# Tcadart/pyLatticeDSO

Hardware: AMD Instinct MI355X
Metric: beams/s assembly+PCG-solve (higher is better)
Workload: dtype f64

## Files before the change

### pylatticedso_amd/csrc/pl_coarse.h

```cpp
#pragma once
#include <hip/hip_runtime.h>

#include <algorithm>
#include <cstdint>
#include <cstdlib>
#include <vector>

#include "pl_dense.h"
#include "pl_kernels.h"
#include "pl_nodeword.h"
#include "pl_tile.h"

namespace pl {

constexpr int kDclMax = 256;
constexpr int kDclSlots = 4096;
inline bool node_words_enabled() {
  const char *e = std::getenv("PL_NODE_WORDS");
  return !(e && e[0] == '0');
}

struct Coarse {
  bool enabled = false;
  bool ready = false;
// ... 1380 lines not shown
                                                                 const double *__restrict__ xyz,
                                                                 const int32_t *__restrict__ agg_of_tile,
                                                                 const double *__restrict__ cen,
                                                                 const double *__restrict__ yc,
                                                                 const double *__restrict__ yt ,
                                                                 const uint8_t *__restrict__ fixedbits,
                                                                 PT *__restrict__ p, RT *__restrict__ x,
                                                                 const double *__restrict__ scal,
                                                                 double *__restrict__ scal_next,
                                                                 double *__restrict__ hist, int k,
                                                                 double *__restrict__ rc, int ncp,
                                                                 const int32_t *__restrict__ aggL_of_tile ,
                                                                 const double *__restrict__ cenL,
                                                                 const double *__restrict__ ycL,
                                                                 const uint8_t *__restrict__ shared ,
                                                                 double *__restrict__ rcL, int ncpL,
                                                                 const uint8_t *__restrict__ zero_rows ,
                                                                 int cm = 6,
                                                                 const float *__restrict__ rel32 = nullptr ,
                                                                 const uint32_t *__restrict__ nword = nullptr,
                                                                 const uint32_t *__restrict__ dtab = nullptr,
                                                                 double rscale = 0.0 ) {
  if constexpr (!MULTI) shared = nullptr;
  if constexpr (!MULTI || !LOCAL) aggL_of_tile = nullptr;
  double old, rz_new, pap;
  scalar_read3(scal, S_RZ_OLD, S_RZ_NEW, S_PAP, old, rz_new, pap);
  const double beta = (old != 0.0) ? rz_new / old : 0.0;
  const double alpha = (pap != 0.0) ? old / pap : 0.0;
  if (blockIdx.x == 1 || gridDim.x == 1)
    for (int e = threadIdx.x; e < ncp; e += blockDim.x) rc[e] = 0.0;
  if (aggL_of_tile && (blockIdx.x == 2 || gridDim.x <= 2))
    for (int e = threadIdx.x; e < ncpL; e += blockDim.x) rcL[e] = 0.0;
  if (blockIdx.x == 0 && threadIdx.x < kWave) {
    const int s = threadIdx.x;
    double rr = 0.0;
    for (int q = s; q < kSlots; q += kWave) rr += rc[ncp + q];
    rr = wave_sum(rr);
    if (s == 0) hist[k] = rr;
    for (int q = s; q < kSlots; q += kWave) {
      rc[ncp + q] = 0.0;
      rc[ncp + kSlots + q] = 0.0;
      scal_next[S_RZ_OLD * kSlots + q] = scal[S_RZ_NEW * kSlots + q];
      scal_next[S_RZ_NEW * kSlots + q] = 0.0;
      scal_next[S_PAP * kSlots + q] = 0.0;
    }
  }
  const int t = blockIdx.x;
  const int n0 = tile_start[t], n1 = tile_start[t + 1];
  const int a = agg_of_tile[t];
  const double *y = yc + cm * a;
  double U0 = y[0], U1 = y[1], U2 = y[2], W0 = y[3], W1 = y[4], W2 = y[5];
  double T[TM];
#pragma unroll
  for (int k = 0; k < TM; ++k) T[k] = 0.0;
  if (yt) {
    const double *q = yt + TM * (size_t)t;
#pragma unroll
    for (int k = 0; k < TM; ++k) T[k] = q[k];
    if (!shared) {
      U0 += T[0]; U1 += T[1]; U2 += T[2]; W0 += T[3]; W1 += T[4]; W2 += T[5];
    }
  }
  double ED[6] = {0, 0, 0, 0, 0, 0};
  if constexpr (TM == 12) {
    if (cm == 12) {
#pragma unroll
      for (int k = 0; k < 6; ++k) ED[k] = y[6 + k];
      if (!shared) {
#pragma unroll
        for (int k = 0; k < 6; ++k) {
          T[6 + k] += ED[k];
          ED[k] = 0.0;
        }
      }
    }
  }
  const bool own_t = yt && shared;
  const double c0 = cen[3 * a], c1 = cen[3 * a + 1], c2 = cen[3 * a + 2];
  double L[6] = {0, 0, 0, 0, 0, 0}, l0 = 0.0, l1 = 0.0, l2 = 0.0;
  if (aggL_of_tile) {
    const int aL = aggL_of_tile[t];
#pragma unroll
    for (int q = 0; q < 6; ++q) L[q] = ycL[6 * aL + q];
    l0 = cenL[3 * aL];
    l1 = cenL[3 * aL + 1];
    l2 = cenL[3 * aL + 2];
  }
  for (int64_t i = n0 + threadIdx.x; i < n1; i += blockDim.x) {
    if (zero_rows && zero_rows[i]) continue;
    const uint32_t nw = nword ? nword[i] : 0u;
    double rx, ry, rz;
    if (rscale != 0.0) {
      nword_rel(nw, rscale, rx, ry, rz);
    } else if (rel32) {
      rx = (double)rel32[3 * i];
      ry = (double)rel32[3 * i + 1];
      rz = (double)rel32[3 * i + 2];
    } else {
      rx = xyz[3 * i] - c0;
      ry = xyz[3 * i + 1] - c1;
      rz = xyz[3 * i + 2] - c2;
    }
    double zc[6] = {U0 + (W1 * rz - W2 * ry), U1 + (W2 * rx - W0 * rz), U2 + (W0 * ry - W1 * rx), W0, W1, W2};
    if constexpr (TM == 12) {
     if (shared && cm == 12) {
      zc[0] += ED[0] * rx + 0.5 * (ED[3] * ry + ED[5] * rz);
      zc[1] += ED[1] * ry + 0.5 * (ED[3] * rx + ED[4] * rz);
      zc[2] += ED[2] * rz + 0.5 * (ED[4] * ry + ED[5] * rx);
     }
     if (!(shared && shared[i])) {
      zc[0] += T[6] * rx + 0.5 * (T[9] * ry + T[11] * rz);
      zc[1] += T[7] * ry + 0.5 * (T[9] * rx + T[10] * rz);
      zc[2] += T[8] * rz + 0.5 * (T[10] * ry + T[11] * rx);
     }
    }
    if (own_t && !shared[i]) {
      zc[0] += T[0] + (T[4] * rz - T[5] * ry);
      zc[1] += T[1] + (T[5] * rx - T[3] * rz);
      zc[2] += T[2] + (T[3] * ry - T[4] * rx);
      zc[3] += T[3];
      zc[4] += T[4];
      zc[5] += T[5];
    }
    if (aggL_of_tile && !(shared && shared[i])) {
      const double sx = xyz[3 * i] - l0, sy = xyz[3 * i + 1] - l1, sz = xyz[3 * i + 2] - l2;
      zc[0] += L[0] + (L[4] * sz - L[5] * sy);
      zc[1] += L[1] + (L[5] * sx - L[3] * sz);
      zc[2] += L[2] + (L[3] * sy - L[4] * sx);
      zc[3] += L[3];
      zc[4] += L[4];
      zc[5] += L[5];
    }
    const uint32_t *row = dtab ? dtab + 8 * (nw >> 24) : nullptr;
    const unsigned fb = dtab ? row[6] : (unsigned)fixedbits[i];
    const float2 *d2 = dtab ? reinterpret_cast<const float2 *>(row) : reinterpret_cast<const float2 *>(dinv32 + 6 * i);
#pragma unroll
    for (int q = 0; q < 3; ++q) {
      const double2 rr = load_pair(r, 3 * i + q);
      const float2 dd = d2[q];
      double2 pp = load_pair(p, 3 * i + q);
      double2 xx = load_pair(x, 3 * i + q);
      xx.x += alpha * pp.x;
      xx.y += alpha * pp.y;
      store_pair(x, 3 * i + q, xx);
      const double z0 = dd.x * rr.x + (((fb >> (2 * q)) & 1u) ? 0.0 : zc[2 * q]);
      const double z1 = dd.y * rr.y + (((fb >> (2 * q + 1)) & 1u) ? 0.0 : zc[2 * q + 1]);
      pp.x = z0 + beta * pp.x;
      pp.y = z1 + beta * pp.y;
      store_pair(p, 3 * i + q, pp);
    }
  }
}

template <typename PT, typename RT, int TM>
__global__ __launch_bounds__(kBlock) void k_pcg_direction_flat(int64_t N, const int32_t *__restrict__ tile_of_node,
                                                               const RT *__restrict__ r,
                                                               const float *__restrict__ dinv32,
                                                               const double *__restrict__ xyz,
                                                               const int32_t *__restrict__ agg_of_tile,
                                                               const double *__restrict__ cen,
                                                               const double *__restrict__ yc,
                                                               const double *__restrict__ yt ,
                                                               const uint8_t *__restrict__ fixedbits,
                                                               PT *__restrict__ p, RT *__restrict__ x,
                                                               const double *__restrict__ scal,
                                                               double *__restrict__ scal_next,
                                                               double *__restrict__ hist, int k,
                                                               double *__restrict__ rc, int ncp,
                                                               const int32_t *__restrict__ keep ,
                                                               int cm, const uint8_t *__restrict__ shared ,
                                                               const float *__restrict__ rel32 = nullptr ,
                                                               const uint32_t *__restrict__ nword = nullptr,
                                                               const uint32_t *__restrict__ dtab = nullptr,
                                                               double rscale = 0.0 ) {
  double old, rz_new, pap;
  scalar_read3(scal, S_RZ_OLD, S_RZ_NEW, S_PAP, old, rz_new, pap);
  const double beta = (old != 0.0) ? rz_new / old : 0.0;
  const double alpha = (pap != 0.0) ? old / pap : 0.0;
  if (blockIdx.x == 1 || gridDim.x == 1)
    for (int e = threadIdx.x; e < ncp; e += blockDim.x) rc[e] = 0.0;
  if (blockIdx.x == 0 && threadIdx.x < kWave) {
    const int s = threadIdx.x;
    double rr = 0.0;
    for (int q = s; q < kSlots; q += kWave) rr += rc[ncp + q];
    rr = wave_sum(rr);
    if (s == 0) hist[k] = rr;
    for (int q = s; q < kSlots; q += kWave) {
      rc[ncp + q] = 0.0;
      rc[ncp + kSlots + q] = 0.0;
      scal_next[S_RZ_OLD * kSlots + q] = scal[S_RZ_NEW * kSlots + q];
      scal_next[S_RZ_NEW * kSlots + q] = 0.0;
      scal_next[S_PAP * kSlots + q] = 0.0;
    }
  }
  const int64_t lane_pair = (int64_t)blockIdx.x * blockDim.x + threadIdx.x;
  if (lane_pair >= 3 * N) return;
  const int64_t slot = lane_pair / 3;
  const int q = (int)(lane_pair - 3 * slot);
  const int64_t i = keep ? (int64_t)keep[slot] : slot;
  const int64_t pair = 3 * i + q;
  const int t = tile_of_node[i];
  const int a = agg_of_tile[t];
  const double *y = yc + cm * a;
  double C[12];
#pragma unroll
  for (int m = 0; m < 6; ++m) C[m] = y[m];
#pragma unroll
  for (int m = 6; m < 12; ++m) C[m] = 0.0;
  if constexpr (TM == 12) {
    if (cm == 12) {
#pragma unroll
      for (int m = 6; m < 12; ++m) C[m] = y[m];
    }
  }
  if (yt && !(shared && shared[i])) {
    const double *w = yt + TM * (size_t)t;
#pragma unroll
    for (int m = 0; m < TM; ++m) C[m] += w[m];
  }
  const uint32_t nw = nword ? nword[i] : 0u;
  double rx, ry, rz;
  if (rscale != 0.0) {
    nword_rel(nw, rscale, rx, ry, rz);
  } else if (rel32) {
    rx = (double)rel32[3 * i];
    ry = (double)rel32[3 * i + 1];
    rz = (double)rel32[3 * i + 2];
  } else {
    rx = xyz[3 * i] - cen[3 * a];
    ry = xyz[3 * i + 1] - cen[3 * a + 1];
    rz = xyz[3 * i + 2] - cen[3 * a + 2];
  }
  double zc[6] = {C[0] + (C[4] * rz - C[5] * ry), C[1] + (C[5] * rx - C[3] * rz), C[2] + (C[3] * ry - C[4] * rx),
                  C[3], C[4], C[5]};
  if constexpr (TM == 12) {
    zc[0] += C[6] * rx + 0.5 * (C[9] * ry + C[11] * rz);
    zc[1] += C[7] * ry + 0.5 * (C[9] * rx + C[10] * rz);
    zc[2] += C[8] * rz + 0.5 * (C[10] * ry + C[11] * rx);
  }
  double z0 = q == 0 ? zc[0] : (q == 1 ? zc[2] : zc[4]);
  double z1 = q == 0 ? zc[1] : (q == 1 ? zc[3] : zc[5]);
  const uint32_t *row = dtab ? dtab + 8 * (nw >> 24) : nullptr;
  const unsigned fb = dtab ? row[6] : (unsigned)fixedbits[i];
  const float2 dd = dtab ? reinterpret_cast<const float2 *>(row)[q] : reinterpret_cast<const float2 *>(dinv32)[pair];
  const double2 rr = load_pair(r, pair);
  double2 pp = load_pair(p, pair);
  double2 xx = load_pair(x, pair);
  xx.x += alpha * pp.x;
  xx.y += alpha * pp.y;
  store_pair(x, pair, xx);
  z0 = dd.x * rr.x + (((fb >> (2 * q)) & 1u) ? 0.0 : z0);
  z1 = dd.y * rr.y + (((fb >> (2 * q + 1)) & 1u) ? 0.0 : z1);
  pp.x = z0 + beta * pp.x;
  pp.y = z1 + beta * pp.y;
  store_pair(p, pair, pp);
}

}
```

### pylatticedso_amd/csrc/pl_kernels.h

```cpp
#pragma once
#include "pl_device.h"

namespace pl {

constexpr int kBlock = 256;
constexpr int kWave = 64;
constexpr int kDefaultLPN = 4;
constexpr int kSlots = 64;

__device__ __forceinline__ unsigned xcd_block(unsigned b, unsigned nblk) {
  const unsigned xcd = b & 7u, q = nblk >> 3, r = nblk & 7u;
  const unsigned base = (xcd < r) ? xcd * (q + 1) : r * (q + 1) + (xcd - r) * q;
  return base + (b >> 3);
}

__device__ __forceinline__ double dpp_row_shr_add(double v, const int ctrl_tag) {
  int lo = __double2loint(v), hi = __double2hiint(v);
  switch (ctrl_tag) {
    case 1: lo = __builtin_amdgcn_update_dpp(0, lo, 0x111, 0xf, 0xf, true); hi = __builtin_amdgcn_update_dpp(0, hi, 0x111, 0xf, 0xf, true); break;
    case 2: lo = __builtin_amdgcn_update_dpp(0, lo, 0x112, 0xf, 0xf, true); hi = __builtin_amdgcn_update_dpp(0, hi, 0x112, 0xf, 0xf, true); break;
    case 4: lo = __builtin_amdgcn_update_dpp(0, lo, 0x114, 0xf, 0xf, true); hi = __builtin_amdgcn_update_dpp(0, hi, 0x114, 0xf, 0xf, true); break;
    default: lo = __builtin_amdgcn_update_dpp(0, lo, 0x118, 0xf, 0xf, true); hi = __builtin_amdgcn_update_dpp(0, hi, 0x118, 0xf, 0xf, true); break;
  }
  return v + __hiloint2double(hi, lo);
}
__device__ __forceinline__ double row_sums(double v) {
  v = dpp_row_shr_add(v, 1);
  v = dpp_row_shr_add(v, 2);
  v = dpp_row_shr_add(v, 4);
  return dpp_row_shr_add(v, 8);
}
__device__ __forceinline__ double lane_value(double v, int l) {
  return __hiloint2double(__builtin_amdgcn_readlane(__double2hiint(v), l), __builtin_amdgcn_readlane(__double2loint(v), l));
}
__device__ __forceinline__ double lane_value_dyn(double v, int l) {
  return __hiloint2double(__shfl(__double2hiint(v), l), __shfl(__double2loint(v), l));
}
__device__ __forceinline__ double wave_sum(double v) {
  v = dpp_row_shr_add(v, 1);
  v = dpp_row_shr_add(v, 2);
  v = dpp_row_shr_add(v, 4);
  v = dpp_row_shr_add(v, 8);
  const int lo = __double2loint(v), hi = __double2hiint(v);
  double t = __hiloint2double(__builtin_amdgcn_readlane(hi, 15), __builtin_amdgcn_readlane(lo, 15));
  t += __hiloint2double(__builtin_amdgcn_readlane(hi, 31), __builtin_amdgcn_readlane(lo, 31));
  t += __hiloint2double(__builtin_amdgcn_readlane(hi, 47), __builtin_amdgcn_readlane(lo, 47));
  t += __hiloint2double(__builtin_amdgcn_readlane(hi, 63), __builtin_amdgcn_readlane(lo, 63));
  return t;
}

__device__ __forceinline__ void scalar_add(double *scal, int which, double v) {
  unsafeAtomicAdd(scal + which * kSlots + (blockIdx.x & (kSlots - 1)), v);
}
__device__ __forceinline__ double scalar_read(const double *scal, int which) {
  const int lane = threadIdx.x & 63;
  double v = 0.0;
#pragma unroll
  for (int s = lane; s < kSlots; s += 64) v += scal[which * kSlots + s];
  return wave_sum(v);
}

__device__ __forceinline__ void scalar_read2(const double *scal, int a, int b, double &va, double &vb) {
  static_assert(kSlots == kWave, "one slot per lane");
  const int lane = threadIdx.x & 63;
  const double xa = scal[a * kSlots + lane], xb = scal[b * kSlots + lane];
  va = wave_sum(xa);
  vb = wave_sum(xb);
}
__device__ __forceinline__ void scalar_read3(const double *scal, int a, int b, int c, double &va, double &vb, double &vc) {
  static_assert(kSlots == kWave, "one slot per lane");
  const int lane = threadIdx.x & 63;
  const double xa = scal[a * kSlots + lane], xb = scal[b * kSlots + lane], xc = scal[c * kSlots + lane];
  va = wave_sum(xa);
  vb = wave_sum(xb);
  vc = wave_sum(xc);
}

__device__ __forceinline__ double block_sum(double v, double *smem ) {
  v = wave_sum(v);
  const int lane = threadIdx.x & 63, w = threadIdx.x >> 6;
  if (lane == 0) smem[w] = v;
  __syncthreads();
  double t = 0.0;
  if (threadIdx.x == 0) {
#pragma unroll
    for (int i = 0; i < kBlock / kWave; ++i) t += smem[i];
  }
  return t;
}

__device__ __forceinline__ void load6(const double *__restrict__ p, V3 &u, V3 &t) {
  const double2 *q = reinterpret_cast<const double2 *>(p);
  const double2 a = q[0], b = q[1], c = q[2];
  u = {a.x, a.y, b.x};
  t = {b.y, c.x, c.y};
}
__device__ __forceinline__ void store6(double *__restrict__ p, V3 u, V3 t) {
  double2 *q = reinterpret_cast<double2 *>(p);
  q[0] = {u.x, u.y};
  q[1] = {u.z, t.x};
  q[2] = {t.y, t.z};
}

__device__ __forceinline__ void load6(const float *__restrict__ p, V3 &u, V3 &t) {
  const float2 *q = reinterpret_cast<const float2 *>(p);
  const float2 a = q[0], b = q[1], c = q[2];
  u = {(double)a.x, (double)a.y, (double)b.x};
  t = {(double)b.y, (double)c.x, (double)c.y};
}
__device__ __forceinline__ double2 load_pair(const double *v, int64_t pair) {
  return reinterpret_cast<const double2 *>(v)[pair];
}
__device__ __forceinline__ double2 load_pair(const float *v, int64_t pair) {
  const float2 f = reinterpret_cast<const float2 *>(v)[pair];
  return {(double)f.x, (double)f.y};
}
__device__ __forceinline__ void store_pair(double *v, int64_t pair, double2 a) {
  reinterpret_cast<double2 *>(v)[pair] = a;
}
__device__ __forceinline__ void store_pair(float *v, int64_t pair, double2 a) {
  reinterpret_cast<float2 *>(v)[pair] = {(float)a.x, (float)a.y};
}

__device__ __forceinline__ Record load_record(const Record *__restrict__ rec, int64_t i) {
  const double2 *q = reinterpret_cast<const double2 *>(rec + i);
  const double2 a = q[0], b = q[1], c = q[2], d = q[3];
  Record r;
  r.a = a.x; r.c = a.y; r.e1 = b.x; r.e2 = b.y; r.e3 = c.x; r.dx = c.y; r.dy = d.x; r.dz = d.y;
  return r;
}

__global__ __launch_bounds__(kBlock) void k_build_records(int64_t B, const double *__restrict__ xyz,
                                                          const int32_t *__restrict__ conn,
                                                          const double *__restrict__ radius,
                                                          const double *__restrict__ seg_len,
                                                          const int32_t *__restrict__ seg_nsub,
                                                          const double *__restrict__ mult, Material m,
                                                          Record *__restrict__ rec, double *__restrict__ rec5) {
  const int64_t b = (int64_t)xcd_block(blockIdx.x, gridDim.x) * kBlock + threadIdx.x;
  if (b >= B) return;
  if (mult) m = scaled(m, mult[b]);
  const int ia = conn[2 * b], ib = conn[2 * b + 1];
  const V3 d = {xyz[3 * (int64_t)ib] - xyz[3 * (int64_t)ia], xyz[3 * (int64_t)ib + 1] - xyz[3 * (int64_t)ia + 1],
                xyz[3 * (int64_t)ib + 2] - xyz[3 * (int64_t)ia + 2]};
  const double len[3] = {seg_len[3 * b], seg_len[3 * b + 1], seg_len[3 * b + 2]};
  const int ns[3] = {seg_nsub[3 * b], seg_nsub[3 * b + 1], seg_nsub[3 * b + 2]};
  const Flex f = strut_flexibility(radius[b], len, ns, m);
  const Record r = make_record(scalars_from_flex(f), d);
  rec[b] = r;
  if (rec5) {
    double *q = rec5 + 5 * b;
    q[0] = r.a; q[1] = r.c; q[2] = r.e1; q[3] = r.e2; q[4] = r.e3;
  }
}

__global__ __launch_bounds__(kBlock) void k_spmv_atomic(int64_t B, const int32_t *__restrict__ conn,
                                                        const Record *__restrict__ rec, const double *__restrict__ x,
                                                        double *__restrict__ y) {
  const int64_t b = (int64_t)xcd_block(blockIdx.x, gridDim.x) * kBlock + threadIdx.x;
  if (b >= B) return;
  const int64_t ia = conn[2 * b], ib = conn[2 * b + 1];
  const Record r = load_record(rec, b);
  V3 uA, tA, uB, tB, F, M;
  load6(x + 6 * ia, uA, tA);
  load6(x + 6 * ib, uB, tB);
  tip_force(r, uA, tA, uB, tB, F, M);
  const V3 d = {r.dx, r.dy, r.dz};
  const V3 MA = (-1.0) * M - cross(d, F);
  double *ya = y + 6 * ia, *yb = y + 6 * ib;
  unsafeAtomicAdd(yb + 0, F.x); unsafeAtomicAdd(yb + 1, F.y); unsafeAtomicAdd(yb + 2, F.z);
  unsafeAtomicAdd(yb + 3, M.x); unsafeAtomicAdd(yb + 4, M.y); unsafeAtomicAdd(yb + 5, M.z);
  unsafeAtomicAdd(ya + 0, -F.x); unsafeAtomicAdd(ya + 1, -F.y); unsafeAtomicAdd(ya + 2, -F.z);
  unsafeAtomicAdd(ya + 3, MA.x); unsafeAtomicAdd(ya + 4, MA.y); unsafeAtomicAdd(ya + 5, MA.z);
}

__global__ __launch_bounds__(kBlock) void k_mask_dot(int64_t n6, const uint8_t *__restrict__ fixed,
                                                     const double *__restrict__ x, double *__restrict__ y,
                                                     double *__restrict__ dot_out) {
  __shared__ double red[kBlock / kWave];
  double acc = 0.0;
  for (int64_t i = (int64_t)blockIdx.x * kBlock + threadIdx.x; i < n6; i += (int64_t)gridDim.x * kBlock) {
    double v = y[i];
    if (fixed && fixed[i]) { v = 0.0; y[i] = 0.0; }
    acc += x[i] * v;
  }
  if (dot_out) {
    const double t = block_sum(acc, red);
    if (threadIdx.x == 0) unsafeAtomicAdd(dot_out + (blockIdx.x & (kSlots - 1)), t);
  }
}

template <int LPN>
__device__ __forceinline__ double lpn_sum(double v) {
#pragma unroll
  for (int o = kWave / LPN; o < kWave; o <<= 1) v += __shfl_xor(v, o, 64);
  return v;
}

template <int LPN, bool MASK, bool DOT>
__global__ __launch_bounds__(kBlock) void k_spmv_gather(int64_t N, const int64_t *__restrict__ slice_ptr,
                                                        const int2 *__restrict__ ent, const Record *__restrict__ rec,
                                                        const uint8_t *__restrict__ fixedbits,
                                                        const double *__restrict__ x, double *__restrict__ y,
                                                        double *__restrict__ dot_out) {
  __shared__ double red[kBlock / kWave];
  const unsigned blk = xcd_block(blockIdx.x, gridDim.x);
  constexpr int kSliceNodes = kWave / LPN;
  const int lane = threadIdx.x & 63, sub = lane / kSliceNodes;
  const int64_t slice = (int64_t)blk * (kBlock / kWave) + (threadIdx.x >> 6);
  const int64_t i = slice * kSliceNodes + (lane & (kSliceNodes - 1));
  double acc = 0.0;
  if (slice * kSliceNodes < N) {
    const bool live = i < N;
    V3 us = {0, 0, 0}, ts = {0, 0, 0};
    if (live) load6(x + 6 * i, us, ts);
    V3 F = {0, 0, 0}, M = {0, 0, 0};
    const int64_t p0 = slice_ptr[slice], p1 = slice_ptr[slice + 1];
#pragma unroll 2
    for (int64_t p = p0 + lane; p < p1; p += 64) {
      const int2 e = ent[p];
      if (e.x >= 0) {
        Record r = load_record(rec, e.y & 0x7fffffff);
        V3 uo, to, f, m;
        load6(x + 6 * (int64_t)e.x, uo, to);
        if (e.y < 0) r = reversed(r);
        tip_force(r, uo, to, us, ts, f, m);
        F = F + f;
        M = M + m;
// ... 465 lines not shown
```

### pylatticedso_amd/csrc/pl_solver.h

```cpp
#pragma once
#include <type_traits>

#include "pl_assembly.h"
#include "pl_schedule.h"
#include "pl_warm.h"

namespace {

int read_slots(pl_context *c, const double *dev, double *sum) {
  double h[pl::kSlots];
  PL_HIP(hipMemcpyAsync(h, dev, sizeof(h), hipMemcpyDeviceToHost, c->stream));
  PL_HIP(hipStreamSynchronize(c->stream));
  *sum = 0.0;
  for (int k = 0; k < pl::kSlots; ++k) *sum += h[k];
  return PL_OK;
}

int solve_begin(pl_context *c, const double *bb_slots, pl_stats_t *st, double *bb, bool *zero) {
  *zero = false;
  const int rc = read_slots(c, bb_slots, bb);
  if (rc) return rc;
  st->b_norm = std::sqrt(*bb);
  st->iterations = 0;
  st->converged = 0;
  st->rel_residual = 0.0;
  if (*bb > 0.0) return PL_OK;
  *zero = true;
  st->converged = 1;
  return std::isnan(*bb) ? fail(PL_ERR_NAN, "NaN in the right-hand side") : PL_OK;
}

inline void converged_at(pl_stats_t *st, int iterations, double stop_reason) {
  st->converged = 1;
  st->iterations = iterations;
  st->info = 0.0;
  st->stop_reason = stop_reason;
}

template <int V>
using Int = std::integral_constant<int, V>;

template <typename F>
inline void with_tile_modes(const pl_context *c, F &&f) {
  if (tile_modes_now(c) == 12) f(Int<12>{});
  else f(Int<6>{});
}
template <typename F>
inline void with_tail_variant(const pl_context *c, F &&f) {
  with_tile_modes(c, [&](auto tm) {
    if (c->coarseL.ready) f(tm, std::true_type{}, std::true_type{});
    else if (c->dist.active) f(tm, std::true_type{}, std::false_type{});
    else f(tm, std::false_type{}, std::false_type{});
  });
}

struct NodeWords {
  const float *rel32;
  const uint32_t *nword, *dtab;
  double rscale;
};
inline NodeWords node_words_of(const pl_context *c) {
  const pl::Coarse &cs = c->coarse;
  const bool words = node_words_apply(c);
  NodeWords nw;
  nw.rel32 = cs.rel_exact ? (const float *)cs.rel32.p : (const float *)nullptr;
  nw.dtab = words && cs.dcl_ready ? (const uint32_t *)cs.dcl_table : (const uint32_t *)nullptr;
  nw.rscale = words && cs.rel_e >= 0 ? std::ldexp(1.0, -cs.rel_e) : 0.0;
  nw.nword = (nw.dtab || nw.rscale != 0.0) ? (const uint32_t *)cs.nword.p : (const uint32_t *)nullptr;
  return nw;
}

template <typename PT, typename RT, int TM, bool MULTI, bool LOCAL>
void launch_update_tile(pl_context *c, Int<TM>, std::bool_constant<MULTI>, std::bool_constant<LOCAL>, const PT *Ap, RT *r,
                        double *scal, double *rc_out, const NodeWords &nw) {
  pl::Coarse &cs = c->coarse, &cl = c->coarseL;
  hipLaunchKernelGGL((pl::k_pcg_update_tile<PT, RT, TM, MULTI, LOCAL>), dim3((unsigned)cs.n_tiles), dim3(cs.vblock), 0,
                     c->stream, c->tile.tile_start.p, cs.agg_of_tile.p, cs.cen.p, c->xyz.p, Ap, cs.dinv32,
                     c->dist.active ? (const double *)c->dist.weight.p : (const double *)nullptr, r, scal, rc_out,
                     cs.tile_level ? (const double *)cs.Bt_inv : (const double *)nullptr, cs.yt,
                     LOCAL ? (const int32_t *)cl.agg_of_tile.p : (const int32_t *)nullptr,
                     LOCAL ? (const double *)cl.cen.p : (const double *)nullptr,
                     MULTI ? (const uint8_t *)c->sharedbits.p : (const uint8_t *)nullptr, LOCAL ? cl.rc : (double *)nullptr,
                     cs.ncp, c->cond_use ? (const uint8_t *)c->cflag.p : (const uint8_t *)nullptr, cs.cm, nw.rel32, nw.nword,
                     nw.dtab, nw.rscale);
}
template <typename PT, typename RT, int TM, bool MULTI, bool LOCAL>
void launch_direction_coarse(pl_context *c, Int<TM>, std::bool_constant<MULTI>, std::bool_constant<LOCAL>, PT *p, RT *x,
                             const RT *r, double *cur, double *nxt, int hist_slot, const NodeWords &nw) {
  pl::Coarse &cs = c->coarse, &cl = c->coarseL;
  hipLaunchKernelGGL((pl::k_pcg_direction_coarse<PT, RT, TM, MULTI, LOCAL>), dim3((unsigned)cs.n_tiles), dim3(cs.vblock), 0,
                     c->stream, c->tile.tile_start.p, r, cs.dinv32, c->xyz.p, cs.agg_of_tile.p, cs.cen.p, cs.yc,
                     cs.tile_level ? (const double *)cs.yt : (const double *)nullptr, c->fixedbits.p, p, x, cur, nxt,
                     c->hist.p, hist_slot, cs.rc, cs.ncp,
                     LOCAL ? (const int32_t *)cl.agg_of_tile.p : (const int32_t *)nullptr,
                     LOCAL ? (const double *)cl.cen.p : (const double *)nullptr,
                     LOCAL ? (const double *)cl.yc : (const double *)nullptr,
                     MULTI ? (const uint8_t *)c->sharedbits.p : (const uint8_t *)nullptr, LOCAL ? cl.rc : (double *)nullptr,
                     LOCAL ? cl.ncp : 0, c->cond_use ? (const uint8_t *)c->cflag.p : (const uint8_t *)nullptr, cs.cm,
                     nw.rel32, nw.nword, nw.dtab, nw.rscale);
}
template <typename PT, typename RT, int TM>
void launch_direction_flat(pl_context *c, Int<TM>, PT *p, RT *x, const RT *r, double *cur, double *nxt, int hist_slot,
                           const NodeWords &nw) {
  pl::Coarse &cs = c->coarse;
  const int64_t n_flat = c->cond_use ? c->N - c->n_cond : c->N;
  hipLaunchKernelGGL((pl::k_pcg_direction_flat<PT, RT, TM>), dim3((unsigned)((3 * n_flat + pl::kBlock - 1) / pl::kBlock)),
                     dim3(pl::kBlock), 0, c->stream, n_flat, cs.tile_of_node.p, r, cs.dinv32, c->xyz.p, cs.agg_of_tile.p,
                     cs.cen.p, cs.yc, cs.tile_level ? (const double *)cs.yt : (const double *)nullptr, c->fixedbits.p, p, x,
                     cur, nxt, c->hist.p, hist_slot, cs.rc, cs.ncp,
                     c->cond_use ? (const int32_t *)c->ckeep.p : (const int32_t *)nullptr, cs.cm,
                     c->dist.active ? (const uint8_t *)c->sharedbits.p : (const uint8_t *)nullptr, nw.rel32, nw.nword, nw.dtab,
                     nw.rscale);
}

template <typename PT, typename RT>
int pcg_tail_coarse_t(pl_context *c, double *cur, double *nxt, int hist_slot, PT *p, const PT *Ap, RT *x, RT *r) {
  pl::Coarse &cs = c->coarse, &cl = c->coarseL;
  const bool useL = cl.ready;
  const NodeWords nw = node_words_of(c);
  with_tail_variant(c, [&](auto tm, auto multi, auto local) { launch_update_tile(c, tm, multi, local, Ap, r, cur, cs.rc, nw); });
  if (useL)
    pl::coarse_apply(cl, cl.rc, cl.tv, cl.yc, cs.rc + cs.ncp + pl::kSlots, (const double *)nullptr, c->stream);
  if (c->dist.active) {
    if (pl::dist_sum_scalars(c->dist, cs.rc, cs.ncp + 2 * pl::kSlots, c->stream))
      return fail(PL_ERR_HIP, "RCCL all-reduce of the coarse residual failed");
  }
  pl::coarse_apply(cs, cs.rc, cs.tv, cs.yc, cur + pl::S_RZ_NEW * pl::kSlots, cs.rc + cs.ncp + pl::kSlots, c->stream);
  if (!useL && sizeof(PT) == 8)
    with_tile_modes(c, [&](auto tm) { launch_direction_flat(c, tm, p, x, (const RT *)r, cur, nxt, hist_slot, nw); });
  else
    with_tail_variant(c, [&](auto tm, auto multi, auto local) {
      launch_direction_coarse(c, tm, multi, local, p, x, (const RT *)r, cur, nxt, hist_slot, nw);
    });
  PL_HIP(hipGetLastError());
  return PL_OK;
}

int pcg_tail_coarse(pl_context *c, double *cur, double *nxt, int hist_slot) {
  return pcg_tail_coarse_t<double, double>(c, cur, nxt, hist_slot, c->p.p, (const double *)c->Ap.p, c->x.p, c->r.p);
}

inline void ddm_precondition(pl_context *c, double *dot, bool restricted = false) {
  if (c->dd2_ready) {
    pl::Coarse &cs = c->dd2;
    const uint8_t *fx = c->have_bc ? (const uint8_t *)c->fixed.p : (const uint8_t *)nullptr;
    if (!restricted)
      hipLaunchKernelGGL(pl::k_ddm_restrict, dim3((unsigned)c->dd2_n_agg), dim3(pl::kBlock), 0, c->stream, c->dd2_ptr.p,
                         c->dd2_nodes.p, (const double *)c->dd2_cen.p, (const double *)c->dd2_xyz.p, fx,
                         (const double *)c->r.p, cs.rc);
    pl::coarse_apply(cs, cs.rc, cs.tv, cs.yc, dot, (const double *)nullptr, c->stream);
    hipLaunchKernelGGL(pl::k_ddm_two_level_apply, dim3(grid_for(c->N * 6)), dim3(pl::kBlock), 0, c->stream, c->N,
                       (const double *)c->dd_B.p, c->dd2_agg.p, (const double *)c->dd2_cen.p, (const double *)c->dd2_xyz.p, fx,
                       (const double *)cs.yc, (const double *)c->r.p, c->z.p, dot, cs.rc, cs.ncp);
    return;
  }
  if (c->dd_ready)
    pl::dense_apply(c->dd_W.p, c->dd_Wt.p, c->dd_n, c->dd_n, c->r.p, c->dd_tv.p, c->z.p, dot, (const double *)nullptr,
                    c->stream);
  else
    hipLaunchKernelGGL(pl::k_ddm_node_blocks_apply, dim3(grid_for(c->N * 6)), dim3(pl::kBlock), 0, c->stream, c->N,
                       (const double *)c->dd_B.p, (const double *)c->r.p, c->z.p, dot);
}

inline int small_set_size() { return pl::S_COUNT * pl::kSlots; }
inline double *small_set(pl_context *c, int k) { return c->small_scal.p + (size_t)((k + 4) & 3) * small_set_size(); }
inline double *small_rc(pl_context *c, int parity) { return c->small_rc.p + (size_t)(parity & 1) * (c->coarse.ncp + 2 * pl::kSlots); }

int small_prepare(pl_context *c) {
  const int64_t n6 = c->N * 6;
  const size_t nrc = 2 * (size_t)(c->coarse.ncp + 2 * pl::kSlots);
  if (!c->p2.p || c->p2.n < (size_t)n6) PL_HIP(c->p2.alloc((size_t)n6));
  if (!c->small_scal.p) PL_HIP(c->small_scal.alloc(4 * (size_t)small_set_size()));
  if (!c->small_rc.p || c->small_rc.n < nrc) PL_HIP(c->small_rc.alloc(nrc));
  PL_HIP(hipMemsetAsync(c->small_scal.p, 0, 4 * (size_t)small_set_size() * sizeof(double), c->stream));
  PL_HIP(hipMemsetAsync(c->small_rc.p, 0, nrc * sizeof(double), c->stream));
  PL_HIP(hipMemsetAsync(c->p.p, 0, n6 * sizeof(double), c->stream));
  PL_HIP(hipMemsetAsync(c->p2.p, 0, n6 * sizeof(double), c->stream));
  return PL_OK;
}

template <int TM>
void launch_small_z(pl_context *c, Int<TM>, int k, int hist_slot) {
  pl::Coarse &cs = c->coarse;
  hipLaunchKernelGGL((pl::k_small_z<TM>), dim3((unsigned)cs.n_tiles), dim3(cs.vblock), 0, c->stream, c->tile.tile_start.p,
                     cs.agg_of_tile.p, cs.cen.p, c->xyz.p, (const double *)c->r.p, cs.dinv32, c->fixedbits.p,
                     c->cond_use ? (const uint8_t *)c->cflag.p : (const uint8_t *)nullptr, (const float *)cs.Ainv, cs.ncp, cs.cm,
                     (const double *)small_rc(c, k + 1), small_rc(c, k),
                     cs.tile_level ? (const double *)cs.yt : (const double *)nullptr, c->z.p, small_set(c, k + 1),
                     small_set(c, k + 2), c->hist.p, hist_slot);
}
int small_tail(pl_context *c, int k, int hist_slot) {
  const NodeWords none = {(const float *)nullptr, (const uint32_t *)nullptr, (const uint32_t *)nullptr, 0.0};
  with_tile_modes(c, [&](auto tm) {
    launch_update_tile(c, tm, std::false_type{}, std::false_type{}, (const double *)c->Ap.p, c->r.p, small_set(c, k),
                       small_rc(c, k + 1), none);
    launch_small_z(c, tm, k, hist_slot);
  });
  PL_HIP(hipGetLastError());
  return PL_OK;
}

inline double *small_p_of(pl_context *c, int k) { return (k & 1) ? c->p2.p : c->p.p; }

int small_iteration(pl_context *c, int k) {
  pl::Defer df;
  df.z = c->z.p;
  df.p_old = small_p_of(c, k - 1);
  df.p_new = small_p_of(c, k);
  df.xsol = c->x.p;
  df.sc_prev = small_set(c, k - 1);
  df.sc_cur = small_set(c, k);
  double *dot = small_set(c, k) + pl::S_PAP * pl::kSlots;
  const bool stream_form = !c->pal_lds;
  const uint32_t *vw = stream_form ? c->vword_dir.p : c->vword.p;
  const void *tab = stream_form ? (const void *)c->tile.dir_table.p : (const void *)c->pal_dense.p;
  const int n_tab = stream_form ? c->tile.n_dir : c->pal_entries;
  const pl::Rec5 *r5 = stream_form ? reinterpret_cast<const pl::Rec5 *>(c->rec5.p) : (const pl::Rec5 *)nullptr;
  if (c->cond_use) {
    const pl::CondSolve cs = cond_solve(c, pl::kEndsCondensedSolve);
    if (!pl::launch_tile_spmv_lds_defer(c->tile, vw, tab, n_tab, r5, nullptr, df.p_new, nullptr, c->stream,
                                        pl::kEndsCondensedSolve, c->cflag.p, cs, df))
      return fail(PL_ERR_STATE, "short iteration: the LDS-resident K*p does not fit this lattice");
    int rc = launch_spmv(c, df.p_new, c->Ap.p, true, dot, c->maskC.p, pl::kEndsOthers);
    if (rc) return rc;
  } else {
    if (!pl::launch_tile_spmv_lds_defer(c->tile, vw, tab, n_tab, r5, c->fixedbits.p, c->Ap.p, dot, c->stream, pl::kEndsAll,
                                        nullptr, pl::CondSolve(), df))
      return fail(PL_ERR_STATE, "short iteration: the LDS-resident K*p does not fit this lattice");
  }
  return small_tail(c, k, k);
}

int small_finish(pl_context *c, int K) {
  if (K <= 0) return PL_OK;
  hipLaunchKernelGGL(pl::k_small_final_x, dim3(grid_stream(c->N * 6)), dim3(pl::kBlock), 0, c->stream, c->N,
                     c->cond_use ? (const uint8_t *)c->cflag.p : (const uint8_t *)nullptr,
                     (const double *)small_p_of(c, K - 1), (const double *)small_set(c, K - 1), c->x.p);
  PL_HIP(hipGetLastError());
  return PL_OK;
}

inline void periodic_average(pl_context *c, double *v) {
  if (c->n_per_groups > 0)
    hipLaunchKernelGGL(pl::k_periodic_average, dim3(grid_for(6 * c->n_per_groups)), dim3(pl::kBlock), 0, c->stream,
                       c->n_per_groups, c->per_ptr.p, c->per_nodes.p, v);
}

int pcg_iteration(pl_context *c, int k) {
  if (c->small_use) return small_iteration(c, k);
  const int64_t n6 = c->N * 6;
  const int set = pl::S_COUNT * pl::kSlots;
  double *cur = c->scal.p + (k & 1) * set, *nxt = c->scal.p + ((k + 1) & 1) * set;
  int rc = apply_operator(c, c->p.p, c->Ap.p, cur + pl::S_PAP * pl::kSlots);
  if (rc) return rc;
  if (c->coarse.ready) return pcg_tail_coarse(c, cur, nxt, k);
  periodic_average(c, c->Ap.p);
  const bool ref = ref_cg(c) && !c->dist.active;
  const bool restart = ref && c->opt.restart_every > 0 && k > 0 && (k % c->opt.restart_every) == 0;
  const bool has_M = c->dd_ready || c->dd_blocks || c->opt.precond >= 1;
  const double *pn = c->p.p, *psrc = nullptr;
  if (restart) {
    if (has_M) {
      PL_HIP(hipMemcpyAsync(c->tmp.p, c->z.p, n6 * sizeof(double), hipMemcpyDeviceToDevice, c->stream));
      pn = psrc = c->tmp.p;
    } else {
      pn = nullptr;
      psrc = c->z.p;
    }
  }
  const int hcap = ref ? c->hist_cap : 0;
  int *stop = c->stop_use ? c->stop_flag.p : (int *)nullptr;
  const double stop_mintol = ref ? c->opt.mintol : 0.0;
  const double *pn_upd = ref ? pn : (const double *)nullptr;
  const auto update = [&] {
    const auto kern = ref ? pl::k_pcg_update<true> : pl::k_pcg_update<false>;
    hipLaunchKernelGGL(kern, dim3(grid_stream(n6 / 2)), dim3(pl::kBlock), 0, c->stream, n6, c->p.p, c->Ap.p, c->dinv.p,
                       c->x.p, c->r.p, c->z.p, cur, c->opt.alpha_max, pn_upd, (const int *)stop);
  };
  const auto direction = [&]() -> int {
    hipLaunchKernelGGL(pl::k_pcg_direction, dim3(grid_stream(n6 / 2)), dim3(pl::kBlock), 0, c->stream, n6, c->z.p,
                       c->p.p, cur, nxt, c->hist.p, k, psrc, hcap, stop, c->stop_thresh, stop_mintol);
    PL_HIP(hipGetLastError());
    return PL_OK;
// ... 580 lines not shown
```

Before: 256.4 million.

## Specialize flat PCG direction kernel and load tile coefficients via wave-uniform scalar loads

The flat PCG direction kernel is templated on arm source, dtab, tile-level, keep and shared flags, which removes runtime branches and pointer checks. The per-tile coarse coefficients are now fetched through a waterfall loop over the distinct tiles in each wave, using constant-address-space (scalar) loads instead of per-lane vector gathers. Global loads of r/p/x and the scalar slots are issued earlier, before the reductions, and the slot-reset bookkeeping moves to the end of the kernel. Tail lanes are clamped rather than returning early, so the wave-wide ballot stays valid. This adds host-side template instantiations, and the waterfall loop can cost more when a wave spans many tiles.

```diff
diff --git a/pylatticedso_amd/csrc/pl_coarse.h b/pylatticedso_amd/csrc/pl_coarse.h
--- a/pylatticedso_amd/csrc/pl_coarse.h
+++ b/pylatticedso_amd/csrc/pl_coarse.h
@@ -1556,7 +1556,36 @@
   }
 }
 
-template <typename PT, typename RT, int TM>
+constexpr int kArmsBytes = 0, kArmsRel32 = 1, kArmsXyz = 2;
+template <typename T>
+using uniform_ptr = const __attribute__((address_space(4))) T *;
+template <int TM, bool YT>
+__device__ __forceinline__ void flat_coefficients(int tt, uniform_ptr<int32_t> agg_of_tile, uniform_ptr<double> yc,
+                                                  uniform_ptr<double> yt, int cm, bool add_tile, int &a, double (&C)[12]) {
+  a = agg_of_tile[tt];
+  uniform_ptr<double> y = yc + cm * a;
+#pragma unroll
+  for (int m = 0; m < 6; ++m) C[m] = y[m];
+#pragma unroll
+  for (int m = 6; m < 12; ++m) C[m] = 0.0;
+  if constexpr (TM == 12) {
+    const bool strains = cm == 12;
+    uniform_ptr<double> ys = y + (strains ? 6 : 0);
+#pragma unroll
+    for (int m = 0; m < 6; ++m) {
+      const double v = ys[m];
+      C[6 + m] = strains ? v : 0.0;
+    }
+  }
+  if constexpr (YT) {
+    uniform_ptr<double> w = yt + TM * (size_t)tt;
+    if (add_tile) {
+#pragma unroll
+      for (int m = 0; m < TM; ++m) C[m] += w[m];
+    }
+  }
+}
+template <typename PT, typename RT, int TM, int ARMS, bool DTAB, bool YT, bool KEEP, bool SHARED>
 __global__ __launch_bounds__(kBlock) void k_pcg_direction_flat(int64_t N, const int32_t *__restrict__ tile_of_node,
                                                                const RT *__restrict__ r,
                                                                const float *__restrict__ dinv32,
@@ -1573,68 +1602,83 @@
                                                                double *__restrict__ rc, int ncp,
                                                                const int32_t *__restrict__ keep ,
                                                                int cm, const uint8_t *__restrict__ shared ,
-                                                               const float *__restrict__ rel32 = nullptr ,
-                                                               const uint32_t *__restrict__ nword = nullptr,
-                                                               const uint32_t *__restrict__ dtab = nullptr,
-                                                               double rscale = 0.0 ) {
-  double old, rz_new, pap;
-  scalar_read3(scal, S_RZ_OLD, S_RZ_NEW, S_PAP, old, rz_new, pap);
-  const double beta = (old != 0.0) ? rz_new / old : 0.0;
-  const double alpha = (pap != 0.0) ? old / pap : 0.0;
-  if (blockIdx.x == 1 || gridDim.x == 1)
-    for (int e = threadIdx.x; e < ncp; e += blockDim.x) rc[e] = 0.0;
-  if (blockIdx.x == 0 && threadIdx.x < kWave) {
-    const int s = threadIdx.x;
-    double rr = 0.0;
-    for (int q = s; q < kSlots; q += kWave) rr += rc[ncp + q];
-    rr = wave_sum(rr);
-    if (s == 0) hist[k] = rr;
-    for (int q = s; q < kSlots; q += kWave) {
-      rc[ncp + q] = 0.0;
-      rc[ncp + kSlots + q] = 0.0;
-      scal_next[S_RZ_OLD * kSlots + q] = scal[S_RZ_NEW * kSlots + q];
-      scal_next[S_RZ_NEW * kSlots + q] = 0.0;
-      scal_next[S_PAP * kSlots + q] = 0.0;
-    }
-  }
-  const int64_t lane_pair = (int64_t)blockIdx.x * blockDim.x + threadIdx.x;
-  if (lane_pair >= 3 * N) return;
-  const int64_t slot = lane_pair / 3;
-  const int q = (int)(lane_pair - 3 * slot);
-  const int64_t i = keep ? (int64_t)keep[slot] : slot;
+                                                               const float *__restrict__ rel32 ,
+                                                               const uint32_t *__restrict__ nword,
+                                                               const uint32_t *__restrict__ dtab ,
+                                                               double rscale ) {
+  const int64_t pair0 = (int64_t)blockIdx.x * kBlock;
+  const int64_t slot0 = pair0 / 3;
+  const int local = (int)(pair0 - 3 * slot0) + (int)threadIdx.x;
+  const bool live = pair0 + threadIdx.x < 3 * N;
+  const int64_t slot = live ? slot0 + local / 3 : N - 1;
+  const int q = live ? local % 3 : 2;
+  const int64_t i = KEEP ? (int64_t)keep[slot] : slot;
   const int64_t pair = 3 * i + q;
+  const ScalarSlots3 slots = scalar_slots3(scal, S_RZ_OLD, S_RZ_NEW, S_PAP);
   const int t = tile_of_node[i];
-  const int a = agg_of_tile[t];
-  const double *y = yc + cm * a;
-  double C[12];
-#pragma unroll
-  for (int m = 0; m < 6; ++m) C[m] = y[m];
-#pragma unroll
-  for (int m = 6; m < 12; ++m) C[m] = 0.0;
-  if constexpr (TM == 12) {
-    if (cm == 12) {
-#pragma unroll
-      for (int m = 6; m < 12; ++m) C[m] = y[m];
-    }
-  }
-  if (yt && !(shared && shared[i])) {
-    const double *w = yt + TM * (size_t)t;
-#pragma unroll
-    for (int m = 0; m < TM; ++m) C[m] += w[m];
-  }
-  const uint32_t nw = nword ? nword[i] : 0u;
+  const uint32_t nw = (ARMS == kArmsBytes || DTAB) ? nword[i] : 0u;
+  const double2 rr = load_pair(r, pair);
+  double2 pp = load_pair(p, pair);
+  double2 xx = load_pair(x, pair);
+  bool own = true;
+  if constexpr (SHARED) own = !shared[i];
   double rx, ry, rz;
-  if (rscale != 0.0) {
+  if constexpr (ARMS == kArmsBytes) {
     nword_rel(nw, rscale, rx, ry, rz);
-  } else if (rel32) {
+  } else if constexpr (ARMS == kArmsRel32) {
     rx = (double)rel32[3 * i];
     ry = (double)rel32[3 * i + 1];
     rz = (double)rel32[3 * i + 2];
   } else {
-    rx = xyz[3 * i] - cen[3 * a];
-    ry = xyz[3 * i + 1] - cen[3 * a + 1];
-    rz = xyz[3 * i + 2] - cen[3 * a + 2];
-  }
+    rx = xyz[3 * i];
+    ry = xyz[3 * i + 1];
+    rz = xyz[3 * i + 2];
+  }
+  unsigned fb;
+  float2 dd;
+  if constexpr (!DTAB) {
+    fb = (unsigned)fixedbits[i];
+    dd = reinterpret_cast<const float2 *>(dinv32)[pair];
+  }
+  if constexpr (DTAB) {
+    const uint32_t *row = dtab + 8 * (nw >> 24);
+    fb = row[6];
+    dd = reinterpret_cast<const float2 *>(row)[q];
+  }
+  double C[12], cx = 0.0, cy = 0.0, cz = 0.0;
+#pragma unroll
+  for (int m = 0; m < 12; ++m) C[m] = 0.0;
+  uint64_t rest = __builtin_amdgcn_ballot_w64(true);
+  do {
+    const int t0 = __builtin_amdgcn_readlane(t, (int)__builtin_ctzll(rest));
+    int t0_seen = t0;
+    asm volatile("" : "+s"(t0_seen));
+    const bool mine = t == t0_seen;
+    int a0;
+    double C0[12];
+    flat_coefficients<TM, YT>(t0, (uniform_ptr<int32_t>)agg_of_tile, (uniform_ptr<double>)yc, (uniform_ptr<double>)yt, cm, own,
+                              a0, C0);
+    if (mine) {
+#pragma unroll
+      for (int m = 0; m < 12; ++m) C[m] = C0[m];
+      if constexpr (ARMS == kArmsXyz) {
+        uniform_ptr<double> ce = (uniform_ptr<double>)cen + 3 * a0;
+        cx = ce[0];
+        cy = ce[1];
+        cz = ce[2];
+      }
+    }
+    rest &= ~__builtin_amdgcn_ballot_w64(mine);
+  } while (rest != 0);
+  if constexpr (ARMS == kArmsXyz) {
+    rx -= cx;
+    ry -= cy;
+    rz -= cz;
+  }
+  double old, rz_new, pap;
+  scalar_sum3(slots, old, rz_new, pap);
+  const double beta = (old != 0.0) ? rz_new / old : 0.0;
+  const double alpha = (pap != 0.0) ? old / pap : 0.0;
   double zc[6] = {C[0] + (C[4] * rz - C[5] * ry), C[1] + (C[5] * rx - C[3] * rz), C[2] + (C[3] * ry - C[4] * rx),
                   C[3], C[4], C[5]};
   if constexpr (TM == 12) {
@@ -1644,20 +1688,32 @@
   }
   double z0 = q == 0 ? zc[0] : (q == 1 ? zc[2] : zc[4]);
   double z1 = q == 0 ? zc[1] : (q == 1 ? zc[3] : zc[5]);
-  const uint32_t *row = dtab ? dtab + 8 * (nw >> 24) : nullptr;
-  const unsigned fb = dtab ? row[6] : (unsigned)fixedbits[i];
-  const float2 dd = dtab ? reinterpret_cast<const float2 *>(row)[q] : reinterpret_cast<const float2 *>(dinv32)[pair];
-  const double2 rr = load_pair(r, pair);
-  double2 pp = load_pair(p, pair);
-  double2 xx = load_pair(x, pair);
   xx.x += alpha * pp.x;
   xx.y += alpha * pp.y;
-  store_pair(x, pair, xx);
   z0 = dd.x * rr.x + (((fb >> (2 * q)) & 1u) ? 0.0 : z0);
   z1 = dd.y * rr.y + (((fb >> (2 * q + 1)) & 1u) ? 0.0 : z1);
   pp.x = z0 + beta * pp.x;
   pp.y = z1 + beta * pp.y;
-  store_pair(p, pair, pp);
-}
-
-}
+  if (live) {
+    store_pair(x, pair, xx);
+    store_pair(p, pair, pp);
+  }
+  if (blockIdx.x == 1 || gridDim.x == 1)
+    for (int e = threadIdx.x; e < ncp; e += blockDim.x) rc[e] = 0.0;
+  if (blockIdx.x == 0 && threadIdx.x < kWave) {
+    const int s = threadIdx.x;
+    double sum = 0.0;
+    for (int e = s; e < kSlots; e += kWave) sum += rc[ncp + e];
+    sum = wave_sum(sum);
+    if (s == 0) hist[k] = sum;
+    for (int e = s; e < kSlots; e += kWave) {
+      rc[ncp + e] = 0.0;
+      rc[ncp + kSlots + e] = 0.0;
+      scal_next[S_RZ_OLD * kSlots + e] = scal[S_RZ_NEW * kSlots + e];
+      scal_next[S_RZ_NEW * kSlots + e] = 0.0;
+      scal_next[S_PAP * kSlots + e] = 0.0;
+    }
+  }
+}
+
+}
diff --git a/pylatticedso_amd/csrc/pl_kernels.h b/pylatticedso_amd/csrc/pl_kernels.h
--- a/pylatticedso_amd/csrc/pl_kernels.h
+++ b/pylatticedso_amd/csrc/pl_kernels.h
@@ -67,13 +67,21 @@
   va = wave_sum(xa);
   vb = wave_sum(xb);
 }
-__device__ __forceinline__ void scalar_read3(const double *scal, int a, int b, int c, double &va, double &vb, double &vc) {
+struct ScalarSlots3 {
+  double a, b, c;
+};
+__device__ __forceinline__ ScalarSlots3 scalar_slots3(const double *scal, int a, int b, int c) {
   static_assert(kSlots == kWave, "one slot per lane");
   const int lane = threadIdx.x & 63;
-  const double xa = scal[a * kSlots + lane], xb = scal[b * kSlots + lane], xc = scal[c * kSlots + lane];
-  va = wave_sum(xa);
-  vb = wave_sum(xb);
-  vc = wave_sum(xc);
+  return {scal[a * kSlots + lane], scal[b * kSlots + lane], scal[c * kSlots + lane]};
+}
+__device__ __forceinline__ void scalar_sum3(const ScalarSlots3 &s, double &va, double &vb, double &vc) {
+  va = wave_sum(s.a);
+  vb = wave_sum(s.b);
+  vc = wave_sum(s.c);
+}
+__device__ __forceinline__ void scalar_read3(const double *scal, int a, int b, int c, double &va, double &vb, double &vc) {
+  scalar_sum3(scalar_slots3(scal, a, b, c), va, vb, vc);
 }
 
 __device__ __forceinline__ double block_sum(double v, double *smem ) {
diff --git a/pylatticedso_amd/csrc/pl_solver.h b/pylatticedso_amd/csrc/pl_solver.h
--- a/pylatticedso_amd/csrc/pl_solver.h
+++ b/pylatticedso_amd/csrc/pl_solver.h
@@ -44,6 +44,11 @@
 inline void with_tile_modes(const pl_context *c, F &&f) {
   if (tile_modes_now(c) == 12) f(Int<12>{});
   else f(Int<6>{});
+}
+template <typename F>
+inline void with_flag(bool b, F &&f) {
+  if (b) f(std::true_type{});
+  else f(std::false_type{});
 }
 template <typename F>
 inline void with_tail_variant(const pl_context *c, F &&f) {
@@ -104,13 +109,31 @@
                            const NodeWords &nw) {
   pl::Coarse &cs = c->coarse;
   const int64_t n_flat = c->cond_use ? c->N - c->n_cond : c->N;
-  hipLaunchKernelGGL((pl::k_pcg_direction_flat<PT, RT, TM>), dim3((unsigned)((3 * n_flat + pl::kBlock - 1) / pl::kBlock)),
-                     dim3(pl::kBlock), 0, c->stream, n_flat, cs.tile_of_node.p, r, cs.dinv32, c->xyz.p, cs.agg_of_tile.p,
-                     cs.cen.p, cs.yc, cs.tile_level ? (const double *)cs.yt : (const double *)nullptr, c->fixedbits.p, p, x,
-                     cur, nxt, c->hist.p, hist_slot, cs.rc, cs.ncp,
-                     c->cond_use ? (const int32_t *)c->ckeep.p : (const int32_t *)nullptr, cs.cm,
-                     c->dist.active ? (const uint8_t *)c->sharedbits.p : (const uint8_t *)nullptr, nw.rel32, nw.nword, nw.dtab,
-                     nw.rscale);
+  auto go = [&](auto arms, auto dt, auto yt, auto keep, auto sh) {
+    hipLaunchKernelGGL((pl::k_pcg_direction_flat<PT, RT, TM, decltype(arms)::value, decltype(dt)::value, decltype(yt)::value,
+                                                 decltype(keep)::value, decltype(sh)::value>),
+                       dim3((unsigned)((3 * n_flat + pl::kBlock - 1) / pl::kBlock)), dim3(pl::kBlock), 0, c->stream, n_flat,
+                       cs.tile_of_node.p, r, cs.dinv32, c->xyz.p, cs.agg_of_tile.p, cs.cen.p, cs.yc,
+                       cs.tile_level ? (const double *)cs.yt : (const double *)nullptr, c->fixedbits.p, p, x, cur, nxt,
+                       c->hist.p, hist_slot, cs.rc, cs.ncp,
+                       c->cond_use ? (const int32_t *)c->ckeep.p : (const int32_t *)nullptr, cs.cm,
+                       c->dist.active ? (const uint8_t *)c->sharedbits.p : (const uint8_t *)nullptr, nw.rel32, nw.nword,
+                       nw.dtab, nw.rscale);
+  };
+  auto with_arms = [&](auto &&f) {
+    if (nw.rscale != 0.0) f(Int<pl::kArmsBytes>{});
+    else if (nw.rel32) f(Int<pl::kArmsRel32>{});
+    else f(Int<pl::kArmsXyz>{});
+  };
+  with_arms([&](auto arms) {
+    with_flag(nw.dtab != nullptr, [&](auto dt) {
+      with_flag(cs.tile_level, [&](auto yt) {
+        with_flag(c->cond_use, [&](auto keep) {
+          with_flag(c->dist.active, [&](auto sh) { go(arms, dt, yt, keep, sh); });
+        });
+      });
+    });
+  });
 }
 
 template <typename PT, typename RT>
@@ -126,9 +149,14 @@
       return fail(PL_ERR_HIP, "RCCL all-reduce of the coarse residual failed");
   }
   pl::coarse_apply(cs, cs.rc, cs.tv, cs.yc, cur + pl::S_RZ_NEW * pl::kSlots, cs.rc + cs.ncp + pl::kSlots, c->stream);
-  if (!useL && sizeof(PT) == 8)
-    with_tile_modes(c, [&](auto tm) { launch_direction_flat(c, tm, p, x, (const RT *)r, cur, nxt, hist_slot, nw); });
-  else
+  bool flat = false;
+  if constexpr (sizeof(PT) == 8) {
+    if (!useL) {
+      flat = true;
+      with_tile_modes(c, [&](auto tm) { launch_direction_flat(c, tm, p, x, (const RT *)r, cur, nxt, hist_slot, nw); });
+    }
+  }
+  if (!flat)
     with_tail_variant(c, [&](auto tm, auto multi, auto local) {
       launch_direction_coarse(c, tm, multi, local, p, x, (const RT *)r, cur, nxt, hist_slot, nw);
     });
```

Result: faster. 263.4 million (median of 6 runs) (+2.7%).
